# pandegroup/openmm

Measured on NVIDIA H100. Metric: ns/day, higher is better.
Workload: dtype f32

## Files before the change

### openmm_b200/csrc/engine.cu

```cuda
#include "engine.h"
#include "../../include/b200md.h"
#include <stdexcept>
#include <algorithm>
#include <cmath>
#include <cstring>
#include <cstdlib>
#include <map>
#include <set>
#include <dlfcn.h>
#include <thread>

static std::string g_create_error;

template <class T> struct DevBuf {
    T* p = nullptr; size_t n = 0; bool owned = true;
    void attach(void* ptr, size_t count) { free(); p = (T*) ptr; n = count; owned = false; }
    void alloc(size_t count) {
        if (!owned) { if (count > n) throw std::runtime_error("window buffer too small"); return; }
        free(); n = count; if (count) CUDA_CHECK(cudaMalloc(&p, count*sizeof(T)));
    }
    void upload(const std::vector<T>& v) { if (v.size() > n) alloc(v.size()); if (!v.empty()) CUDA_CHECK(cudaMemcpy(p, v.data(), v.size()*sizeof(T), cudaMemcpyHostToDevice)); }
    void zero() { if (n) CUDA_CHECK(cudaMemset(p, 0, n*sizeof(T))); }
    void free() { if (p && owned) cudaFree(p); p = nullptr; n = 0; owned = true; }
    ~DevBuf() { free(); }
// ... 19 lines not shown
        AllReduce = (decltype(AllReduce)) dlsym(lib, "ncclAllReduce");
        AllGather = (decltype(AllGather)) dlsym(lib, "ncclAllGather");
        CommDestroy = (decltype(CommDestroy)) dlsym(lib, "ncclCommDestroy");
        GetErrorString = (decltype(GetErrorString)) dlsym(lib, "ncclGetErrorString");
        if (!GetUniqueId || !CommInitRank || !AllReduce) { err = "libnccl lacks required symbols"; return false; }
        return true;
    }
};
static NcclApi g_nccl;
enum { NCCL_INT8 = 0, NCCL_INT64 = 4, NCCL_FLOAT32 = 7, NCCL_FLOAT64 = 8, NCCL_SUM = 0 };

struct b200md_ctx {
    int device = 0;
    int natoms = 0, npad = 0, nblocks = 0;
    bool finalized = false;
    std::string err;
    cudaStream_t stream = nullptr;
    cudaStream_t streamPme = nullptr;
    cudaStream_t streamBonded = nullptr;
    cudaEvent_t evFork = nullptr, evJoin = nullptr, evJoinBonded = nullptr;
    bool pmeOnly = false;
    bool listDirty = true;
    bool overlapPme = true;
    bool pmeBrick = true;
    int brickAtoms = 64, brickPoints = 8192;
    bool listBuilt = false;
    std::vector<double> mass, charge, sigma, epsilon;
    b200md_nonbonded_desc nbdesc{};
    bool haveNb = false;
    std::vector<int> excI, excJ; std::vector<double> excQQ, excSig, excEps;
    std::vector<int> bondI, bondJ; std::vector<double> bondR0, bondK;
    std::vector<int> angI, angJ, angK; std::vector<double> angT0, angKK;
    std::vector<int> torI, torJ, torK, torL, torN; std::vector<double> torPhase, torKK;
    std::vector<int> rbI, rbJ, rbK, rbL; std::vector<double> rbC;
    std::vector<int> cmapSize, cmapMap, cmapAtoms; std::vector<double> cmapCoeff;
    std::vector<unsigned char> bondGroup, angGroup, torGroup, rbGroup, cmapGroup;
    std::vector<int> conI, conJ; std::vector<double> conD;
    int cmFreq = 0;
    std::vector<int4> hUnitAtoms;
    double boxA[3] = {0, 0, 0}, boxB[3] = {0, 0, 0}, boxC[3] = {0, 0, 0};
    bool haveBox = false;
    bool haveOrigin = false;
    double padFrac = 0.10;
    DevBuf<float4> posq, velm, sposq[2], swrap[2], refPos, atomShift, blockCenter[2], blockHalf[2], superCenter[2], superHalf[2];
    DevBuf<float2> sigeps, ssigeps[2];
    DevBuf<double> chargeD; DevBuf<double2> sigepsD;
    DevBuf<long long> force;
    DevBuf<double> energy, cmScratch;
    DevBuf<int> molStart, molAtoms, cellOffset, sorig[2], sortedOf, cellRank, cellCount, cellFill, atomCell, tmpSorted, tileI[2], tileJ[2], tileMask[2], listCounters, counters, exclStart, exclList;
    DevBuf<unsigned int> maskPool[2];
    DevBuf<unsigned long long> stepCounter;
    DevBuf<unsigned int> blocksDone;
    bool stepStateValid = false;
    DevBuf<real> grid, eterm;
    DevBuf<long long> gridFixed;
    DevBuf<real2> cgrid;
    DevBuf<real2> tw[3];
    DevBuf<double> moduli[3];
    DevBuf<int2> bondAtoms, excAtoms; DevBuf<double2> bondParams, angleParams;
    DevBuf<int4> angleAtoms, torsionAtoms, unitAtoms; DevBuf<double4> torsionParams, excParams;
    DevBuf<int> unitType; DevBuf<float4> unitParams;
    DevBuf<unsigned char> bondGroupDev, angGroupDev, torGroupDev, rbGroupDev, cmapGroupDev;
    DevBuf<int4> rbAtoms, cmapAtomsDev; DevBuf<double> rbParams, cmapCoeffDev; DevBuf<int> cmapMapDev; DevBuf<int2> cmapMapsDev;
    std::vector<int> ccmaCons;
    DevBuf<int> ccCompCon, ccCompAtom, ccRowStart, ccCol, ccAtoms, ccAStart, ccACon;
    DevBuf<int2> ccConAtoms; DevBuf<float> ccDist, ccRedMass, ccVal, ccDelta1, ccDelta2;
    DevBuf<float4> ccRij, ccXold, ccXunc;
    int precision = B200MD_PRECISION_SINGLE;
    DevBuf<float4> posqCorr; DevBuf<double4> velmD, unitParamsD;
    DevBuf<double> ccDistD, ccRedMassD, ccDelta1D, ccDelta2D; DevBuf<double4> ccRijD, ccXoldD, ccXuncD, ccXposD;
    bool mixed() const { return precision == B200MD_PRECISION_MIXED; }
    CcmaDev ccma{};
    NbDev nb{};
    PmeDev pme{};
    BondedDev bd{};
    UnitDev units{};
    IntegDev integ{};
    bool haveIntegrator = false;
    double dt = 0, temperature = 0, friction = 0;
    double time = 0;
    int64_t stepCount = 0;
    double selfEnergy = 0, dispersionCoefficient = 0;
    int64_t forceEvals = 0, kernelLaunches = 0, graphInstantiations = 0;
    DevBuf<int> baroStart, baroAtoms;
    int baroNmol = 0;
    DevBuf<float4> savePosq, savePosqCorr; DevBuf<int> saveCellOffset; DevBuf<long long> saveForce;
    bool haveSaved = false;
    cudaGraphExec_t stepGraph = nullptr;
    cudaGraphExec_t multiGraph = nullptr;
    bool graphValid = false;
    bool multiValid = false;
    bool useGraph = true;
    int graphSteps = 8;
    int stepLaunches = 0;
    void* comm = nullptr;
    int rank = 0, world = 1;
    bool p2p = false;
    CommDev cd{};
    char* window = nullptr; size_t windowBytes = 0;
    void* peerMapped[B200MD_MAX_RANKS] = {nullptr};
    DevBuf<unsigned long long> commCounters;
    DevBuf<unsigned int> commDone;
    bool velStale = false;
    std::vector<float4> hbuf4, hcorr4;
    std::vector<int> hoffset;
    std::vector<long long> hforce;
};

#define API_BEGIN(ctx) if (!(ctx)) return -1; try { CUDA_CHECK(cudaSetDevice((ctx)->device));
#define API_END(ctx) } catch (std::exception& e) { (ctx)->err = e.what(); return -1; } return 0;

static void require(bool cond, const char* msg) { if (!cond) throw std::runtime_error(msg); }
static void check_flags(b200md_ctx* c);
static void sync_velocities(b200md_ctx* c);
static void sync_positions(b200md_ctx* c);

extern "C" const char* b200md_version(void) { return "b200md 0.2 (sm_90a)"; }
extern "C" const char* b200md_last_error(const b200md_ctx* ctx) { return ctx ? ctx->err.c_str() : g_create_error.c_str(); }

extern "C" int b200md_create(b200md_ctx** out, int device, int natoms) {
    try {
        require(out != nullptr && natoms > 0, "b200md_create: bad arguments");
        int count = 0;
        cudaError_t e = cudaGetDeviceCount(&count);
        if (e != cudaSuccess || count == 0)
            throw std::runtime_error(std::string("b200md_create: no CUDA device available (") + cudaGetErrorString(e) + "); this library has no CPU fallback");
        require(device >= 0 && device < count, "b200md_create: device index out of range");
        CUDA_CHECK(cudaSetDevice(device));
        b200md_ctx* c = new b200md_ctx();
        c->device = device;
        c->natoms = natoms;
        c->npad = ((natoms + 31)/32)*32;
        c->nblocks = c->npad/32;
        CUDA_CHECK(cudaStreamCreateWithFlags(&c->stream, cudaStreamNonBlocking));
        if (getenv("B200MD_NO_OVERLAP")) c->overlapPme = false;
        if (getenv("B200MD_PME_BRICK")) c->pmeBrick = atoi(getenv("B200MD_PME_BRICK")) != 0;
        if (getenv("B200MD_PME_BRICK_POINTS")) c->brickPoints = std::max(1, atoi(getenv("B200MD_PME_BRICK_POINTS")));
        int hi = 0;
        CUDA_CHECK(cudaDeviceGetStreamPriorityRange(nullptr, &hi));
        CUDA_CHECK(cudaStreamCreateWithPriority(&c->streamPme, cudaStreamNonBlocking, hi));
        CUDA_CHECK(cudaStreamCreateWithPriority(&c->streamBonded, cudaStreamNonBlocking, hi));
        CUDA_CHECK(cudaEventCreateWithFlags(&c->evFork, cudaEventDisableTiming));
        CUDA_CHECK(cudaEventCreateWithFlags(&c->evJoin, cudaEventDisableTiming));
        CUDA_CHECK(cudaEventCreateWithFlags(&c->evJoinBonded, cudaEventDisableTiming));
        c->mass.assign(natoms, 1.0);
        c->charge.assign(natoms, 0.0); c->sigma.assign(natoms, 1.0); c->epsilon.assign(natoms, 0.0);
        const char* pf = getenv("B200MD_PAD_FRACTION");
        if (pf) c->padFrac = atof(pf);
        const char* ug = getenv("B200MD_USE_GRAPH");
        if (ug) c->useGraph = atoi(ug) != 0;
        const char* gs = getenv("B200MD_GRAPH_STEPS");
        if (gs) c->graphSteps = std::max(1, atoi(gs));
        *out = c;
        return 0;
    } catch (std::exception& e) { g_create_error = e.what(); return -1; }
}

extern "C" void b200md_destroy(b200md_ctx* ctx) {
    if (!ctx) return;
    cudaSetDevice(ctx->device);
    cudaDeviceSynchronize();
    if (ctx->stepGraph) cudaGraphExecDestroy(ctx->stepGraph);
// ... 1201 lines not shown
        }
        else { CUDA_CHECK(cudaMemcpy(p, ctx->velm.p, sizeof(float4)*ctx->npad, cudaMemcpyDeviceToHost)); p += sizeof(float4)*ctx->npad; }
        CUDA_CHECK(cudaMemcpy(p, ctx->cellOffset.p, sizeof(int)*3*ctx->npad, cudaMemcpyDeviceToHost));
        return need;
    } catch (std::exception& e) { ctx->err = e.what(); return -1; }
}
extern "C" int b200md_checkpoint_load(b200md_ctx* ctx, const void* buf, int64_t size) {
    API_BEGIN(ctx)
    ctx->stepStateValid = false;
    require(ctx->finalized, "checkpoint_load before finalize");
    require(size >= (int64_t) sizeof(CkptHeader), "checkpoint blob too small");
    CkptHeader h; memcpy(&h, buf, sizeof(h));
    require(memcmp(h.magic, "B200MDCK", 8) == 0 && (h.version == 2 || h.version == 3) && h.natoms == ctx->natoms, "checkpoint blob does not match this context");
    require(h.version == ckpt_version(ctx), h.version == 3 ? "the checkpoint was written in mixed precision and this context is single precision"
                                                           : "the checkpoint was written in single precision and this context is mixed precision");
    require(size >= ckpt_bytes(ctx), "checkpoint blob too small");
    sync_positions(ctx);
    CUDA_CHECK(cudaStreamSynchronize(ctx->stream));
    ctx->time = h.time; ctx->stepCount = h.stepCount;
    for (int i = 0; i < 3; i++) { ctx->boxA[i] = h.box[i]; ctx->boxB[i] = h.box[3+i]; ctx->boxC[i] = h.box[6+i]; }
    const char* p = (const char*) buf + sizeof(h);
    CUDA_CHECK(cudaMemcpy(ctx->posq.p, p, sizeof(float4)*ctx->npad, cudaMemcpyHostToDevice)); p += sizeof(float4)*ctx->npad;
    if (ctx->mixed()) {
        CUDA_CHECK(cudaMemcpy(ctx->posqCorr.p, p, sizeof(float4)*ctx->npad, cudaMemcpyHostToDevice)); p += sizeof(float4)*ctx->npad;
        CUDA_CHECK(cudaMemcpy(ctx->velmD.p, p, sizeof(double4)*ctx->npad, cudaMemcpyHostToDevice)); p += sizeof(double4)*ctx->npad;
    }
    else { CUDA_CHECK(cudaMemcpy(ctx->velm.p, p, sizeof(float4)*ctx->npad, cudaMemcpyHostToDevice)); p += sizeof(float4)*ctx->npad; }
    CUDA_CHECK(cudaMemcpy(ctx->cellOffset.p, p, sizeof(int)*3*ctx->npad, cudaMemcpyHostToDevice));
    CUDA_CHECK(cudaMemcpy(ctx->stepCounter.p, &h.rngStep, sizeof(unsigned long long), cudaMemcpyHostToDevice));
    host_set_state(ctx); ctx->velStale = false;
    if (ctx->haveBox) apply_box(ctx);
    const int one = 1;
    CUDA_CHECK(cudaMemcpy(&ctx->counters.p[CT_REBUILD], &one, sizeof(int), cudaMemcpyHostToDevice)); ctx->listDirty = true;
    API_END(ctx)
}

static bool role_split(const b200md_ctx* c) { return c->world > 1 && c->comm && !c->p2p && c->nb.method == B200MD_NB_PME && c->haveNb; }
static NbDev role_nb(const b200md_ctx* c) {
    NbDev nb = c->nb;
    if (role_split(c)) {
        if (c->rank == c->world - 1) { nb.rank = 0; nb.world = 1; }
        else nb.world = c->world - 1;
    }
    return nb;
}

static PmeDev pme_for_launch(const b200md_ctx* c) {
    PmeDev p = c->pme;
    p.brickAtoms = (c->pmeBrick && c->world == 1 && !c->pmeOnly && c->listBuilt) ? c->brickAtoms : 0;
    p.brickPoints = c->brickPoints;
    return p;
}

static int enqueue_forces(b200md_ctx* c, int terms, bool energy, bool forcesAlreadyZero = false, bool inStep = false, unsigned int groupMask = 0xffffffffu) {
    int launches = 0;
    cudaStream_t s = c->stream;
    if (!forcesAlreadyZero) CUDA_CHECK(cudaMemsetAsync(c->force.p, 0, sizeof(long long)*3*c->npad, s));
    if (energy) CUDA_CHECK(cudaMemsetAsync(c->energy.p, 0, sizeof(double)*B200MD_NUM_ENERGY, s));
    bool direct = (terms & B200MD_TERM_NB_DIRECT) && c->haveNb;
    bool recip = (terms & B200MD_TERM_NB_RECIP) && c->haveNb && c->nb.method == B200MD_NB_PME;
    const bool split = role_split(c);
    const int pmeRank = c->world - 1;
    NbDev nbSave = c->nb;
    if (split) {
        if (c->rank == pmeRank) direct = false; else recip = false;
        c->nb = role_nb(c);
    }
    struct Restore { b200md_ctx* c; NbDev saved; ~Restore() { c->nb = saved; } } restore{c, nbSave};
    const bool p2p = c->p2p;
    const bool fork = direct && recip && c->overlapPme && !(c->world > 1 && c->comm && !p2p);
    cudaStream_t sp = fork ? c->streamPme : s;
    if (p2p && !direct) { launch_pos_wait(c->nb, c->cd, s); launches++; }
    const PmeDev pme = pme_for_launch(c);
    const bool forkAfterList = fork && direct && pme.brickAtoms > 0;
    auto launch_recip = [&]() {
        if (fork) {
            CUDA_CHECK(cudaEventRecord(c->evFork, s));
            CUDA_CHECK(cudaStreamWaitEvent(sp, c->evFork, 0));
        }
        if (recip) {
            launch_pme_spread(c->nb, pme, c->cd, sp); launches++;
            if (p2p) { launch_grid_push(c->pme, c->cd, sp); launches++; }
            else if (c->world > 1 && c->comm && !split) {
                int rc = g_nccl.AllReduce(c->gridFixed.p, c->gridFixed.p, (size_t) c->pme.nx*c->pme.ny*c->pme.nz, NCCL_INT64, NCCL_SUM, c->comm, sp);
                if (rc != 0) throw std::runtime_error("ncclAllReduce(grid) failed");
            }
            launch_pme_fft_conv(c->nb, c->pme, c->cd, energy && (split || p2p || c->rank == 0), fft_beside_tiles(c), sp); launches += pme_fft_launch_count(c->pme);
            launch_pme_gather(c->nb, pme, c->cd, sp); launches++;
        }
        if (fork) CUDA_CHECK(cudaEventRecord(c->evJoin, sp));
    };
    if (!forkAfterList) launch_recip();
    if (direct) {
        launch_check_displacement(c->nb, c->cd, s); launches++;
        launch_list_build(c->nb, s); launches += LIST_BUILD_LAUNCHES;
    }
    int bterms = terms & (B200MD_TERM_BONDS | B200MD_TERM_ANGLES | B200MD_TERM_TORSIONS | B200MD_TERM_RB_TORSIONS | B200MD_TERM_CMAP);
    if (c->haveNb) bterms |= terms & B200MD_TERM_NB_DIRECT;
    const int nbonded = c->bd.nbonds + c->bd.nangles + c->bd.ntorsions + c->bd.nrb + c->bd.ncmap + c->bd.nexc;
    const bool bonded = bterms && nbonded > 0 && !(split && c->rank == pmeRank);
    auto launch_bonded_terms = [&](cudaStream_t sb) { BondedDev bd = c->bd; bd.groupMask = groupMask; launch_bonded(c->nb, bd, bterms, energy, sb); launches++; };
    const bool forkBonded = forkAfterList && bonded;
    if (forkAfterList) launch_recip();
    if (forkBonded) {
        CUDA_CHECK(cudaStreamWaitEvent(c->streamBonded, c->evFork, 0));
        launch_bonded_terms(c->streamBonded);
        CUDA_CHECK(cudaEventRecord(c->evJoinBonded, c->streamBonded));
    }
    if (direct) { launch_pair(c->nb, energy, s); launches++; }
    if (bonded && !forkBonded) launch_bonded_terms(s);
    const bool pushEarly = p2p && fork;
    if (pushEarly) { launch_force_push(c->nb, c->cd, s); launches++; }
    if (fork) CUDA_CHECK(cudaStreamWaitEvent(s, c->evJoin, 0));
    if (forkBonded) CUDA_CHECK(cudaStreamWaitEvent(s, c->evJoinBonded, 0));
    if (p2p) {
        if (!pushEarly) { launch_force_push(c->nb, c->cd, s); launches++; }
        if (!inStep) { launch_force_total(c->nb, c->cd, s); launches += 2; }
    }
    if (c->world > 1 && c->comm) {
        int rc = 0;
        if (!p2p) rc = g_nccl.AllReduce(c->force.p, c->force.p, (size_t) 3*c->npad, NCCL_INT64, NCCL_SUM, c->comm, s);
        if (rc != 0) throw std::runtime_error("ncclAllReduce(force) failed");
        if (energy) {
            rc = g_nccl.AllReduce(c->energy.p, c->energy.p, B200MD_NUM_ENERGY, NCCL_FLOAT64, NCCL_SUM, c->comm, s);
            if (rc != 0) throw std::runtime_error("ncclAllReduce(energy) failed");
        }
    }
    CUDA_CHECK(cudaGetLastError());
    return launches;
}

static void check_flags(b200md_ctx* c) {
    if (!c->finalized) return;
    int h[8];
    CUDA_CHECK(cudaMemcpyAsync(h, c->counters.p, sizeof(int)*8, cudaMemcpyDeviceToHost, c->stream));
    CUDA_CHECK(cudaStreamSynchronize(c->stream));
    if (h[CT_OVERFLOW] == 2) throw std::runtime_error("B200 platform: neighbour-list construction timed out at a grid barrier (k_list_prep)");
    if (h[CT_OVERFLOW] == 3) throw std::runtime_error("B200 platform: multi-GPU exchange timed out waiting for a peer rank (every rank must issue the same sequence of calls)");
    if (h[CT_OVERFLOW]) throw std::runtime_error("B200 platform: neighbour-list tile capacity exceeded (" + std::to_string(c->nb.maxTiles) + " tiles) during the preceding steps; the trajectory since the last state read is invalid");
}

static bool role_split(const b200md_ctx* c);
static NbDev role_nb(const b200md_ctx* c);
static void invalidate_graph(b200md_ctx* c);

static void prepare_list(b200md_ctx* c) {
    if (!c->listDirty || !c->haveNb) { c->listDirty = false; return; }
// ... 31 lines not shown

extern "C" int b200md_compute(b200md_ctx* ctx, int terms, int want_forces, double* energy) {
    return b200md_compute_groups(ctx, terms, 0xffffffffu, want_forces, energy);
}

extern "C" int b200md_compute_groups(b200md_ctx* ctx, int terms, unsigned int bonded_group_mask, int want_forces, double* energy) {
    API_BEGIN(ctx)
    ctx->stepStateValid = false;
    (void) want_forces;
    require(ctx->finalized, "compute before finalize");
    const bool wantE = energy != nullptr;
    prepare_list(ctx);
    ctx->kernelLaunches += enqueue_forces(ctx, terms, wantE, false, false, bonded_group_mask);
    ctx->forceEvals++;
    if (wantE) {
        double h[B200MD_NUM_ENERGY];
        CUDA_CHECK(cudaMemcpyAsync(h, ctx->energy.p, sizeof(h), cudaMemcpyDeviceToHost, ctx->stream));
        check_flags(ctx);
        double e = 0;
        if (terms & B200MD_TERM_BONDS) e += h[EN_BOND];
        if (terms & B200MD_TERM_ANGLES) e += h[EN_ANGLE];
        if (terms & B200MD_TERM_TORSIONS) e += h[EN_TORSION];
        if (terms & B200MD_TERM_RB_TORSIONS) e += h[EN_RBTORSION];
        if (terms & B200MD_TERM_CMAP) e += h[EN_CMAP];
        if (ctx->haveNb) {
            if (terms & B200MD_TERM_NB_DIRECT) {
                e += h[EN_NB] + h[EN_EXC];
                const int m = ctx->nb.method;
                if (m == B200MD_NB_CUTOFF_PERIODIC || m == B200MD_NB_PME)
                    e += ctx->dispersionCoefficient/ctx->nb.box.volume;
            }
            if ((terms & B200MD_TERM_NB_RECIP) && ctx->nb.method == B200MD_NB_PME) e += h[EN_RECIP] + ctx->selfEnergy;
        }
        *energy = e;
    }
    API_END(ctx)
}

extern "C" int b200md_set_integrator(b200md_ctx* ctx, int kind, double dt, double temperature, double friction, int seed, double tol) {
    API_BEGIN(ctx)
    require(kind >= 0 && kind <= 2, "unknown integrator kind");
    IntegDev& in = ctx->integ;
    in.kind = kind; in.dt = (float) dt; in.tol = (float) tol; in.seed = (unsigned int) seed;
    const double kT = B200MD_BOLTZ*temperature;
    in.kT = (float) kT;
    const double vscale = std::exp(-dt*friction);
    in.vscale = (float) vscale;
    in.fscale = (float) (friction == 0 ? dt : (1-vscale)/friction);
    in.noisescale = (float) (kind == B200MD_INT_LANGEVIN_MIDDLE ? std::sqrt(1-vscale*vscale) : std::sqrt(kT*(1-vscale*vscale)));
    in.dtD = dt; in.tolD = tol; in.kTD = kT; in.vscaleD = vscale;
    in.fscaleD = friction == 0 ? dt : (1-vscale)/friction;
    in.noisescaleD = kind == B200MD_INT_LANGEVIN_MIDDLE ? std::sqrt(1-vscale*vscale) : std::sqrt(kT*(1-vscale*vscale));
    in.stepCounter = ctx->stepCounter.p;
    in.fused = 0; in.cmEveryStep = 0; in.cmScratch = ctx->cmScratch.p; in.blocksDone = ctx->blocksDone.p;
    ctx->dt = dt; ctx->temperature = temperature; ctx->friction = friction;
    ctx->haveIntegrator = true;
    invalidate_graph(ctx);
    API_END(ctx)
}

static int enqueue_step(b200md_ctx* c) {
    int launches = enqueue_forces(c, B200MD_TERM_ALL, false, true, true);
    IntegDev in = c->integ;
    in.fused = 1;
    in.cmEveryStep = (c->cmFreq == 1) ? 1 : 0;
    in.cmScratch = c->cmScratch.p;
    in.blocksDone = c->blocksDone.p;
    if (c->ccma.ncomp > 0) { launch_ccma_step(c->nb, c->ccma, in, c->stream); launches += 1; }
    launch_integrate(c->nb, c->units, in, c->cd, c->stream); launches += 1;
    return launches;
}

extern "C" int b200md_integrate_only(b200md_ctx* ctx) {
    API_BEGIN(ctx)
    ctx->stepStateValid = false;
    require(ctx->finalized && ctx->haveIntegrator, "integrate before finalize / set_integrator");
    if (ctx->ccma.ncomp > 0) launch_ccma_step(ctx->nb, ctx->ccma, ctx->integ, ctx->stream);
    launch_integrate(ctx->nb, ctx->units, ctx->integ, ctx->cd, ctx->stream);
    ctx->kernelLaunches += 2;
    ctx->velStale = ctx->p2p;
    ctx->time += ctx->dt; ctx->stepCount++;
    CUDA_CHECK(cudaGetLastError());
    API_END(ctx)
}

static void capture_steps(b200md_ctx* c, int nsteps, cudaGraphExec_t* exec, int* launches) {
    cudaGraph_t g;
    CUDA_CHECK(cudaStreamBeginCapture(c->stream, cudaStreamCaptureModeThreadLocal));
    int l = 0;
    try { for (int k = 0; k < nsteps; k++) l += enqueue_step(c); } catch (...) { cudaStreamEndCapture(c->stream, &g); throw; }
    CUDA_CHECK(cudaStreamEndCapture(c->stream, &g));
    *launches = l;
    if (*exec) {
        cudaGraphExecUpdateResultInfo info;
        if (cudaGraphExecUpdate(*exec, g, &info) == cudaSuccess) { cudaGraphDestroy(g); return; }
        (void) cudaGetLastError();
    }
    if (*exec) { cudaGraphExecDestroy(*exec); *exec = nullptr; }
    const cudaError_t e = cudaGraphInstantiate(exec, g, c->world == 1 ? cudaGraphInstantiateFlagUseNodePriority : 0);
    cudaGraphDestroy(g);
    CUDA_CHECK(e);
    c->graphInstantiations++;
}

extern "C" int b200md_step(b200md_ctx* ctx, int nsteps) {
    API_BEGIN(ctx)
    require(ctx->finalized && ctx->haveIntegrator, "step before finalize / set_integrator");
    b200md_ctx* c = ctx;
    int remaining = nsteps;
    prepare_list(c);
    if (!c->stepStateValid) {
        CUDA_CHECK(cudaMemsetAsync(c->force.p, 0, sizeof(long long)*3*c->npad, c->stream));
        if (c->cmFreq == 1) {
            IntegDev in = c->integ;
            in.cmScratch = c->cmScratch.p;
            sync_velocities(c);
            launch_cm_prime(c->nb, in, c->cd, c->stream);
        }
        c->stepStateValid = true;
    }
    while (remaining > 0) {
        if (c->cmFreq > 1 && c->stepCount % c->cmFreq == 0) { sync_velocities(c); launch_remove_cm(c->nb, c->cmScratch.p, c->stream); c->kernelLaunches += 2; }
        int done = 1;
        if (c->useGraph) {
            int untilCm = (c->cmFreq > 1) ? (int) (c->cmFreq - c->stepCount % c->cmFreq) : remaining;
            if (c->graphSteps > 1 && remaining >= c->graphSteps && untilCm >= c->graphSteps) {
                if (!c->multiValid) { int l; capture_steps(c, c->graphSteps, &c->multiGraph, &l); c->stepLaunches = l/c->graphSteps; c->multiValid = true; }
                CUDA_CHECK(cudaGraphLaunch(c->multiGraph, c->stream));
                done = c->graphSteps;
            }
            else {
                if (!c->graphValid) { capture_steps(c, 1, &c->stepGraph, &c->stepLaunches); c->graphValid = true; }
                CUDA_CHECK(cudaGraphLaunch(c->stepGraph, c->stream));
            }
            c->kernelLaunches += (int64_t) c->stepLaunches*done;
        }
        else
            c->kernelLaunches += enqueue_step(c);
        c->velStale = c->p2p;
        c->forceEvals += done;
        c->stepCount += done;
        c->time += c->dt*done;
        remaining -= done;
    }
    CUDA_CHECK(cudaGetLastError());
    API_END(ctx)
}

extern "C" int b200md_kinetic_energy(b200md_ctx* ctx, double* ke) {
    API_BEGIN(ctx)
    require(ctx->finalized, "kinetic_energy before finalize");
    const bool shifted = ctx->haveIntegrator && ctx->integ.kind != B200MD_INT_LANGEVIN_MIDDLE;
    const double shift = !shifted ? 0.0 : ctx->mixed() ? 0.5*ctx->integ.dtD : (double) (0.5f*ctx->integ.dt);
    sync_positions(ctx); sync_velocities(ctx);
    CUDA_CHECK(cudaMemsetAsync(ctx->energy.p + EN_KE, 0, sizeof(double), ctx->stream));
    launch_kinetic_energy(ctx->nb, ctx->units, ctx->integ, shift, ctx->stream);
    launch_ccma_kinetic(ctx->nb, ctx->ccma, shift, 1e-4f, ctx->stream);
    ctx->kernelLaunches++;
    CUDA_CHECK(cudaMemcpyAsync(ke, ctx->energy.p + EN_KE, sizeof(double), cudaMemcpyDeviceToHost, ctx->stream));
    check_flags(ctx);
    API_END(ctx)
}
extern "C" int b200md_apply_constraints(b200md_ctx* ctx, double tol) {
    API_BEGIN(ctx)
    sync_positions(ctx);
    launch_constrain_positions(ctx->nb, ctx->units, tol, ctx->stream);
    launch_ccma_apply(ctx->nb, ctx->ccma, false, tol, ctx->stream);
    ctx->kernelLaunches++;
    CUDA_CHECK(cudaStreamSynchronize(ctx->stream));
    API_END(ctx)
}
extern "C" int b200md_apply_velocity_constraints(b200md_ctx* ctx, double tol) {
    API_BEGIN(ctx)
    ctx->stepStateValid = false;
    sync_positions(ctx); sync_velocities(ctx);
    launch_constrain_velocities(ctx->nb, ctx->units, tol, ctx->stream);
    launch_ccma_apply(ctx->nb, ctx->ccma, true, tol, ctx->stream);
    ctx->kernelLaunches++;
    CUDA_CHECK(cudaStreamSynchronize(ctx->stream));
    API_END(ctx)
}

extern "C" int b200md_comm_unique_id(void* id128) {
    std::string err;
    if (!g_nccl.load(err)) { g_create_error = err; return -1; }
    return g_nccl.GetUniqueId(id128) == 0 ? 0 : -1;
}
extern "C" int b200md_comm_init(b200md_ctx* ctx, int rank, int world, const void* id128) {
    API_BEGIN(ctx)
    require(!ctx->finalized, "comm_init must precede finalize");
    require(!ctx->mixed() || world <= 1, "comm_init: mixed precision is not supported in multi-GPU runs (use Precision=single)");
    std::string err;
    if (!g_nccl.load(err)) throw std::runtime_error(err);
    NcclApi::Uid uid; memcpy(uid.b, id128, 128);
    int rc = g_nccl.CommInitRank(&ctx->comm, world, uid, rank);
    if (rc != 0) throw std::runtime_error(std::string("ncclCommInitRank failed: ") + (g_nccl.GetErrorString ? g_nccl.GetErrorString(rc) : "?"));
    ctx->rank = rank; ctx->world = world;
    DevBuf<long long> warm; warm.alloc(64); warm.zero();
// ... 170 lines not shown
```

### openmm_b200/csrc/engine.h

```cpp
#pragma once
#include <cuda_runtime.h>
#include <stdint.h>
#include <stdexcept>
#include <string>
#include <vector>

#define B200MD_TILE 32
#define B200MD_PME_ORDER 5
#define B200MD_FORCE_SCALE 4294967296.0
#define B200MD_ONE_4PI_EPS0 138.93545764438198
#define B200MD_BOLTZ 0.00831446261815324
#define B200MD_MAX_RADIX 16
#define B200MD_MAX_FFT_STAGES 8

#define CUDA_CHECK(x) do { cudaError_t e_ = (x); if (e_ != cudaSuccess) throw std::runtime_error(std::string(#x) + ": " + cudaGetErrorString(e_)); } while (0)

template <typename... P, typename... A>
inline void launch_high(void (*kernel)(P...), dim3 grid, dim3 block, size_t smem, cudaStream_t s, A... args) {
    static const int hi = [] { int lo = 0, h = 0; cudaDeviceGetStreamPriorityRange(&lo, &h); return h; }();
    cudaLaunchAttribute at[1];
    at[0].id = cudaLaunchAttributePriority;
    at[0].val.priority = hi;
    cudaLaunchConfig_t cfg = {};
    cfg.gridDim = grid; cfg.blockDim = block; cfg.dynamicSmemBytes = smem; cfg.stream = s;
// ... 92 lines not shown
    bool smPartition;
    float closeCut2;
};

enum { EN_NB = 0, EN_RECIP = 1, EN_BOND = 2, EN_ANGLE = 3, EN_TORSION = 4, EN_EXC = 5, EN_KE = 6, EN_RBTORSION = 7, EN_CMAP = 8,
       B200MD_NUM_ENERGY = 9 };

struct PmeDev {
    int nx, ny, nz, nzc;
    real* grid;
    long long* gridFixed;
    real2* cgrid;
    real* eterm;
    const double* moduli[3];
    FftPlanDev plan[3];
    double alpha;
    int brickAtoms;
    int brickPoints;
};

struct BondedDev {
    int nbonds, nangles, ntorsions, nrb, ncmap, nexc;
    const int2* bondAtoms; const double2* bondParams;
    const int4* angleAtoms; const double2* angleParams;
    const int4* torsionAtoms; const double4* torsionParams;
    const int4* rbAtoms; const double* rbParams;
    const int4* cmapAtoms; const int* cmapMap; const int2* cmapMaps; const double* cmapCoeff;
    const int2* excAtoms; const double4* excParams;
    int excPeriodic;
    const unsigned char* bondGroup; const unsigned char* angleGroup; const unsigned char* torsionGroup;
    const unsigned char* rbGroup; const unsigned char* cmapGroup;
    unsigned int groupMask;
};

struct UnitDev {
    int nunits;
    const int4* unitAtoms;
    const int* unitType;
    const float4* unitParams;
    const double4* unitParamsD;
};

struct IntegDev {
    int kind;
    float dt, vscale, fscale, noisescale;
    float kT;
    float tol;
    double dtD, vscaleD, fscaleD, noisescaleD, kTD, tolD;
    unsigned int seed;
    unsigned long long stepIndex;
    unsigned long long* stepCounter;
    int fused;
    int cmEveryStep;
    double* cmScratch;
    unsigned int* blocksDone;
};

#define B200MD_MAX_RANKS 8
enum { CH_POS = 0,
       CH_FORCE = 1,
       CH_FINAL = 2,
       CH_GRID = 3,
       CH_FWD = 4,
       CH_INV = 5,
       CH_POT = 6,
       CH_VEL = 7,
       CH_COUNT = 8 };
struct CommDev {
    int rank, world;
    int atomLo[B200MD_MAX_RANKS + 1];
    int unitLo[B200MD_MAX_RANKS + 1];
    int xLo[B200MD_MAX_RANKS + 1];
    int lineChunk;
    int maxPlanes;
    char* peer[B200MD_MAX_RANKS];
    size_t offFlags, offPosq, offVelm, offForce, offFinbox, offCm, offGridInbox, offLineBuf, offPlaneBuf, offGrid;
    unsigned long long* epoch;
    unsigned long long* posNeed;
    unsigned int* done;
    int* errFlag;
    int posByPush;
};

#ifdef __CUDACC__
__device__ __forceinline__ unsigned long long ld_acquire_sys(const unsigned long long* p) {
    unsigned long long v;
    asm volatile("ld.acquire.sys.global.u64 %0, [%1];" : "=l"(v) : "l"(p) : "memory");
    return v;
}
__device__ __forceinline__ void st_release_sys(unsigned long long* p, unsigned long long v) {
    asm volatile("st.release.sys.global.u64 [%0], %1;" :: "l"(p), "l"(v) : "memory");
}
__device__ __forceinline__ unsigned long long* comm_flag(const CommDev& cd, int onRank, int ch, int src) {
    return (unsigned long long*) (cd.peer[onRank] + cd.offFlags) + ch*B200MD_MAX_RANKS + src;
}
__device__ __forceinline__ void comm_wait(const CommDev& cd, int ch, unsigned long long need) {
    if (cd.world > 1 && need != 0ull) {
        if (threadIdx.x < cd.world && (int) threadIdx.x != cd.rank && threadIdx.y == 0 && threadIdx.z == 0) {
            const unsigned long long* f = comm_flag(cd, cd.rank, ch, threadIdx.x);
            long spins = 0;
            while (ld_acquire_sys(f) < need) {
                if (*((volatile int*) cd.errFlag) == 3) break;
                __nanosleep(64);
                if (++spins > (1L << 22)) { *cd.errFlag = 3; break; }
            }
        }
// ... 191 lines not shown
```

### openmm_b200/csrc/integrate.cu

```cuda
#include "engine.h"
#include <algorithm>
#include "../../include/b200md.h"

template <class R> struct V3 { R x, y, z; };
template <class R> __device__ __forceinline__ V3<R> operator+(V3<R> a, V3<R> b) { return {a.x+b.x, a.y+b.y, a.z+b.z}; }
template <class R> __device__ __forceinline__ V3<R> operator-(V3<R> a, V3<R> b) { return {a.x-b.x, a.y-b.y, a.z-b.z}; }
template <class R> __device__ __forceinline__ V3<R> operator*(V3<R> a, R s) { return {a.x*s, a.y*s, a.z*s}; }
template <class R> __device__ __forceinline__ R dot(V3<R> a, V3<R> b) { return a.x*b.x + a.y*b.y + a.z*b.z; }

template <class R>
__device__ void settle_positions(const V3<R>* x, V3<R>* d, const R* m, R dist1, R dist2) {
    const V3<R> xp0 = d[0], xp1 = d[1], xp2 = d[2];
    const R xb0 = x[1].x-x[0].x, yb0 = x[1].y-x[0].y, zb0 = x[1].z-x[0].z;
    const R xc0 = x[2].x-x[0].x, yc0 = x[2].y-x[0].y, zc0 = x[2].z-x[0].z;
    const R invTotalMass = R(1)/(m[0]+m[1]+m[2]);
    const R xcom = (xp0.x*m[0] + (xb0+xp1.x)*m[1] + (xc0+xp2.x)*m[2])*invTotalMass;
    const R ycom = (xp0.y*m[0] + (yb0+xp1.y)*m[1] + (yc0+xp2.y)*m[2])*invTotalMass;
    const R zcom = (xp0.z*m[0] + (zb0+xp1.z)*m[1] + (zc0+xp2.z)*m[2])*invTotalMass;
    const R xa1 = xp0.x - xcom, ya1 = xp0.y - ycom, za1 = xp0.z - zcom;
    const R xb1 = xb0 + xp1.x - xcom, yb1 = yb0 + xp1.y - ycom, zb1 = zb0 + xp1.z - zcom;
    const R xc1 = xc0 + xp2.x - xcom, yc1 = yc0 + xp2.y - ycom, zc1 = zc0 + xp2.z - zcom;
    const R xaksZd = yb0*zc0 - zb0*yc0, yaksZd = zb0*xc0 - xb0*zc0, zaksZd = xb0*yc0 - yb0*xc0;
    const R xaksXd = ya1*zaksZd - za1*yaksZd, yaksXd = za1*xaksZd - xa1*zaksZd, zaksXd = xa1*yaksZd - ya1*xaksZd;
    const R xaksYd = yaksZd*zaksXd - zaksZd*yaksXd, yaksYd = zaksZd*xaksXd - xaksZd*zaksXd, zaksYd = xaksZd*yaksXd - yaksZd*xaksXd;
// ... 111 lines not shown
    V3<R> x[4], v[4], f[4];
    R invM[4], m[4];
    R4<R> prm;
};

template <class R> __device__ R4<R> unit_params(const UnitDev& un, int u);
template <> __device__ __forceinline__ float4 unit_params<float>(const UnitDev& un, int u) { return un.unitParams[u]; }
template <> __device__ __forceinline__ double4 unit_params<double>(const UnitDev& un, int u) { return un.unitParamsD[u]; }

template <class R>
__device__ __forceinline__ bool load_unit(const NbDev& nb, const UnitDev& un, int u, Unit<R>& U, bool wantForce, const CommDev* cd = nullptr) {
    const int4 at = un.unitAtoms[u];
    U.atom[0] = at.x; U.atom[1] = at.y; U.atom[2] = at.z; U.atom[3] = at.w;
    U.type = un.unitType[u];
    U.prm = unit_params<R>(un, u);
    U.n = 0;
#pragma unroll
    for (int k = 0; k < 4; k++) {
        const int a = U.atom[k];
        if (a < 0) continue;
        U.n = k+1;
        const R4<R> p = load_pos<R>(nb, a);
        const R4<R> v = vel_array<R>(nb)[a];
        U.x[k] = {p.x, p.y, p.z};
        U.v[k] = {v.x, v.y, v.z};
        U.invM[k] = v.w;
        U.m[k] = (v.w > R(0)) ? R(1)/v.w : R(0);
        if (wantForce) {
            long long fx = nb.force[a], fy = nb.force[a + nb.npad], fz = nb.force[a + 2*nb.npad];
            if (cd != nullptr && cd->world > 1) {
                const long long* in = (const long long*) (cd->peer[cd->rank] + cd->offFinbox);
                for (int q = 0; q < cd->world; q++) if (q != cd->rank) {
                    const long long* iq = in + (size_t) q*3*nb.npad;
                    fx += iq[a]; fy += iq[a + nb.npad]; fz += iq[a + 2*nb.npad];
                }
            }
            U.f[k] = {fixed_to_real<R>(fx), fixed_to_real<R>(fy), fixed_to_real<R>(fz)};
        }
    }
    return true;
}

template <class R>
__device__ __forceinline__ void constrain_pos(const Unit<R>& U, V3<R>* d, R tol) {
    if (U.type == 1) settle_positions(U.x, d, U.m, U.prm.x, U.prm.y);
    else if (U.type == 2) { const R dist[3] = {U.prm.x, U.prm.y, U.prm.z}; shake_positions(U.x, d, U.invM, dist, U.n-1, tol); }
}
template <class R>
__device__ __forceinline__ void constrain_vel(const Unit<R>& U, V3<R>* v, R tol) {
    if (U.type == 1) settle_velocities(U.x, v, U.m);
    else if (U.type == 2) shake_velocities(U.x, v, U.invM, U.n-1, tol);
}

template <int KIND, class R>
__global__ void __launch_bounds__(128, sizeof(R) == 8 ? 1 : 0) k_integrate(NbDev nb, UnitDev un, IntegDev in, CommDev cd) {
    const bool multi = cd.world > 1;
    const bool useInbox = multi && in.fused;
    const unsigned long long E = multi ? *cd.epoch + 1ull : 0ull;
    if (useInbox) comm_wait(cd, CH_FORCE, E);
    const int u = (multi ? cd.unitLo[cd.rank] : 0) + blockIdx.x*blockDim.x + threadIdx.x;
    const bool active = u < (multi ? cd.unitLo[cd.rank + 1] : un.nunits);
    const unsigned long long step = *in.stepCounter;
    const IntegR<R> ic = integ_r<R>(in);
    Unit<R> U;
    U.n = 0;
    V3<R> d[4];
    const R invDt = R(1)/ic.dt;
    const bool cmFused = in.fused && in.cmEveryStep;
    V3<R> vcm = {R(0), R(0), R(0)};
    if (cmFused) {
        double c[4];
        if (multi) {
            const double* t = (const double*) (cd.peer[cd.rank] + cd.offCm) + 4*(step % 3ull);
            c[0] = c[1] = c[2] = c[3] = 0.0;
            for (int q = 0; q < cd.world; q++) for (int k = 0; k < 4; k++) c[k] += t[q*12 + k];
        }
        else { const double* t = in.cmScratch + 4*(step % 3ull); c[0] = t[0]; c[1] = t[1]; c[2] = t[2]; c[3] = t[3]; }
        const double im = (c[3] > 0.0) ? 1.0/c[3] : 0.0;
        vcm = {(R) (c[0]*im), (R) (c[1]*im), (R) (c[2]*im)};
    }
    if (active) {
    load_unit(nb, un, u, U, true, useInbox ? &cd : nullptr);
    if (in.fused) {
        _Pragma("unroll") for (int k = 0; k < 4; k++) if (k < U.n) {
            const int a = U.atom[k];
            nb.force[a] = 0; nb.force[a + nb.npad] = 0; nb.force[a + 2*nb.npad] = 0;
            if (U.invM[k] > R(0)) U.v[k] = U.v[k] - vcm;
        }
    }
    if (KIND == B200MD_INT_LANGEVIN_MIDDLE) {
        _Pragma("unroll") for (int k = 0; k < 4; k++) if (k < U.n) U.v[k] = U.v[k] + U.f[k]*(ic.dt*U.invM[k]);
        constrain_vel(U, U.v, ic.tol);
        V3<R> du[4];
        _Pragma("unroll") for (int k = 0; k < 4; k++) if (k < U.n) {
            d[k] = U.v[k]*(R(0.5)*ic.dt);
            if (U.invM[k] > R(0)) {
                const float3 g = gauss3(in.seed, U.atom[k], step);
                const R ns = ic.noisescale*sqrt_r(ic.kT*U.invM[k]);
                U.v[k] = U.v[k]*ic.vscale + V3<R>{g.x, g.y, g.z}*ns;
            }
            d[k] = d[k] + U.v[k]*(R(0.5)*ic.dt);
            if (U.invM[k] == R(0)) d[k] = {R(0), R(0), R(0)};
            du[k] = d[k];
        }
        constrain_pos(U, d, ic.tol);
        _Pragma("unroll") for (int k = 0; k < 4; k++) if (k < U.n) U.v[k] = U.v[k] + (d[k] - du[k])*invDt;
    }
    else {
        _Pragma("unroll") for (int k = 0; k < 4; k++) if (k < U.n) {
            V3<R> vn;
            if (KIND == B200MD_INT_LANGEVIN) {
                vn = U.v[k]*ic.vscale + U.f[k]*(ic.fscale*U.invM[k]);
                if (U.invM[k] > R(0) && ic.noisescale > R(0)) {
                    const float3 g = gauss3(in.seed, U.atom[k], step);
                    vn = vn + V3<R>{g.x, g.y, g.z}*(ic.noisescale*sqrt_r(U.invM[k]));
                }
            }
            else
                vn = U.v[k] + U.f[k]*(ic.dt*U.invM[k]);
            if (U.invM[k] == R(0)) vn = U.v[k];
            d[k] = (U.invM[k] == R(0)) ? V3<R>{R(0), R(0), R(0)} : vn*ic.dt;
        }
        constrain_pos(U, d, ic.tol);
        _Pragma("unroll") for (int k = 0; k < 4; k++) if (k < U.n) if (U.invM[k] > R(0)) U.v[k] = d[k]*invDt;
    }
    _Pragma("unroll") for (int k = 0; k < 4; k++) if (k < U.n) {
        const int a = U.atom[k];
        store_pos<R>(nb, a, U.x[k].x + d[k].x, U.x[k].y + d[k].y, U.x[k].z + d[k].z);
        vel_array<R>(nb)[a] = make_r4(U.v[k].x, U.v[k].y, U.v[k].z, U.invM[k]);
        if (multi && !cd.posByPush) {
            const float4 pn = nb.posq[a];
            for (int k = 1; k < cd.world; k++) {
                const int q = (cd.rank + k) % cd.world;
                ((float4*) (cd.peer[q] + cd.offPosq))[a] = pn;
            }
        }
    }
    }
    if (!in.fused && !(multi && !cd.posByPush)) return;
    if (cmFused) {
        double px = 0, py = 0, pz = 0, m = 0;
        _Pragma("unroll") for (int k = 0; k < 4; k++) if (k < U.n && U.invM[k] > R(0)) {
            const double mk = U.m[k];
            px += mk*U.v[k].x; py += mk*U.v[k].y; pz += mk*U.v[k].z; m += mk;
        }
        for (int off = 16; off > 0; off >>= 1) {
            px += __shfl_xor_sync(0xffffffffu, px, off); py += __shfl_xor_sync(0xffffffffu, py, off);
            pz += __shfl_xor_sync(0xffffffffu, pz, off); m += __shfl_xor_sync(0xffffffffu, m, off);
        }
        __shared__ double red[4][4];
        if ((threadIdx.x & 31) == 0) { red[threadIdx.x >> 5][0] = px; red[threadIdx.x >> 5][1] = py; red[threadIdx.x >> 5][2] = pz; red[threadIdx.x >> 5][3] = m; }
        __syncthreads();
        if (threadIdx.x < 4) {
            double t = 0;
            for (int w = 0; w < (int) (blockDim.x >> 5); w++) t += red[w][threadIdx.x];
            atomicAdd(&in.cmScratch[4*((step + 1ull) % 3ull) + threadIdx.x], t);
            if (blockIdx.x == 0) in.cmScratch[4*((step + 2ull) % 3ull) + threadIdx.x] = 0.0;
        }
    }
    if (multi && !cd.posByPush) {
        const bool lastBlock = comm_arrive(cd, CH_POS, gridDim.x);
        if (lastBlock && threadIdx.x == 0) {
            if (cmFused) {
                const double* mine = in.cmScratch + 4*((step + 1ull) % 3ull);
                for (int q = 0; q < cd.world; q++) {
                    double* t = (double*) (cd.peer[q] + cd.offCm) + cd.rank*12 + 4*((step + 1ull) % 3ull);
                    for (int k = 0; k < 4; k++) t[k] = ((volatile const double*) mine)[k];
                }
            }
            comm_publish(cd, CH_POS, E);
            *cd.posNeed = E;
            *cd.epoch = E;
            *in.stepCounter = step + 1ull;
        }
        return;
    }
    __shared__ int last;
    __syncthreads();
    if (threadIdx.x == 0) {
        __threadfence();
        last = (atomicAdd(in.blocksDone, 1u) == gridDim.x - 1);
    }
    __syncthreads();
    if (last && threadIdx.x == 0) {
        *in.blocksDone = 0u;
        *in.stepCounter = step + 1ull;
    }
}

__global__ void k_step_advance(IntegDev in) { *in.stepCounter += 1ull; }

template <class R>
__global__ void __launch_bounds__(256) k_cm_prime(NbDev nb, IntegDev in, double* table) {
    const unsigned long long step = *in.stepCounter;
    double* c = table + 4*(step % 3ull);
    const int a = blockIdx.x*blockDim.x + threadIdx.x;
    double px = 0, py = 0, pz = 0, m = 0;
    if (a < nb.natoms) {
        const R4<R> v = vel_array<R>(nb)[a];
        if (v.w > R(0)) { m = 1.0/v.w; px = m*v.x; py = m*v.y; pz = m*v.z; }
    }
    for (int off = 16; off > 0; off >>= 1) {
        px += __shfl_xor_sync(0xffffffffu, px, off); py += __shfl_xor_sync(0xffffffffu, py, off);
        pz += __shfl_xor_sync(0xffffffffu, pz, off); m += __shfl_xor_sync(0xffffffffu, m, off);
    }
    __shared__ double red[8][4];
    if ((threadIdx.x & 31) == 0) { red[threadIdx.x >> 5][0] = px; red[threadIdx.x >> 5][1] = py; red[threadIdx.x >> 5][2] = pz; red[threadIdx.x >> 5][3] = m; }
    __syncthreads();
    if (threadIdx.x < 4) {
        double t = 0;
        for (int w = 0; w < 8; w++) t += red[w][threadIdx.x];
        atomicAdd(&c[threadIdx.x], t);
    }
}

void launch_cm_prime(const NbDev& nb, const IntegDev& integ, const CommDev& cd, cudaStream_t s) {
    cudaMemsetAsync(integ.cmScratch, 0, 12*sizeof(double), s);
    double* table = integ.cmScratch;
    if (cd.world > 1) {
        table = (double*) (cd.peer[cd.rank] + cd.offCm);
        cudaMemsetAsync(table, 0, (size_t) B200MD_MAX_RANKS*12*sizeof(double), s);
    }
    if (nb.velmD) k_cm_prime<double><<<(nb.natoms + 255)/256, 256, 0, s>>>(nb, integ, table);
    else k_cm_prime<float><<<(nb.natoms + 255)/256, 256, 0, s>>>(nb, integ, table);
}

template <int KIND>
static void launch_integrate_kind(int grid, const NbDev& nb, const UnitDev& units, const IntegDev& integ, const CommDev& cd, cudaStream_t s) {
    if (nb.velmD) k_integrate<KIND, double><<<grid, 64, 0, s>>>(nb, units, integ, cd);
    else k_integrate<KIND, float><<<grid, 64, 0, s>>>(nb, units, integ, cd);
}

void launch_integrate(const NbDev& nb, const UnitDev& units, const IntegDev& integ, const CommDev& cd, cudaStream_t s) {
    const int n = cd.world > 1 ? cd.unitLo[cd.rank + 1] - cd.unitLo[cd.rank] : units.nunits;
    const int grid = std::max(1, (n + 63)/64);
    if (integ.kind == B200MD_INT_VERLET) launch_integrate_kind<B200MD_INT_VERLET>(grid, nb, units, integ, cd, s);
    else if (integ.kind == B200MD_INT_LANGEVIN) launch_integrate_kind<B200MD_INT_LANGEVIN>(grid, nb, units, integ, cd, s);
    else launch_integrate_kind<B200MD_INT_LANGEVIN_MIDDLE>(grid, nb, units, integ, cd, s);
    if (!integ.fused && (cd.world <= 1 || cd.posByPush)) k_step_advance<<<1, 1, 0, s>>>(integ);
// ... 155 lines not shown
```

Baseline: 1341.

## Fold neighbor-list displacement check into the integrate kernel

Moves the per-step displacement check and sorted-position refresh into the integration kernel, which runs per constraint unit, whenever there is a single rank, a nonbonded force and no CCMA. In-step force evaluation then skips its separate check-displacement launch. One standalone check still runs at the start of each step call, and the last block resets the list counters. This removes a kernel launch and a pass over positions each step, at the cost of extra work in the integrator and a more fragile coupling of list state to it.

```diff
diff --git a/openmm_b200/csrc/engine.cu b/openmm_b200/csrc/engine.cu
--- a/openmm_b200/csrc/engine.cu
+++ b/openmm_b200/csrc/engine.cu
@@ -95,6 +95,7 @@
     DevBuf<unsigned long long> stepCounter;
     DevBuf<unsigned int> blocksDone;
     bool stepStateValid = false;
+    bool listChecked = false;
     DevBuf<real> grid, eterm;
     DevBuf<long long> gridFixed;
     DevBuf<real2> cgrid;
@@ -150,7 +151,7 @@
     std::vector<long long> hforce;
 };
 
-#define API_BEGIN(ctx) if (!(ctx)) return -1; try { CUDA_CHECK(cudaSetDevice((ctx)->device));
+#define API_BEGIN(ctx) if (!(ctx)) return -1; (ctx)->listChecked = false; try { CUDA_CHECK(cudaSetDevice((ctx)->device));
 #define API_END(ctx) } catch (std::exception& e) { (ctx)->err = e.what(); return -1; } return 0;
 
 static void require(bool cond, const char* msg) { if (!cond) throw std::runtime_error(msg); }
@@ -1458,6 +1459,10 @@
     return p;
 }
 
+static bool fold_check(const b200md_ctx* c) {
+    return c->world == 1 && c->haveNb && c->ccma.ncomp == 0;
+}
+
 static int enqueue_forces(b200md_ctx* c, int terms, bool energy, bool forcesAlreadyZero = false, bool inStep = false, unsigned int groupMask = 0xffffffffu) {
     int launches = 0;
     cudaStream_t s = c->stream;
@@ -1498,7 +1503,7 @@
     };
     if (!forkAfterList) launch_recip();
     if (direct) {
-        launch_check_displacement(c->nb, c->cd, s); launches++;
+        if (!(inStep && fold_check(c))) { launch_check_displacement(c->nb, c->cd, s); launches++; }
         launch_list_build(c->nb, s); launches += LIST_BUILD_LAUNCHES;
     }
     int bterms = terms & (B200MD_TERM_BONDS | B200MD_TERM_ANGLES | B200MD_TERM_TORSIONS | B200MD_TERM_RB_TORSIONS | B200MD_TERM_CMAP);
@@ -1636,7 +1641,7 @@
     in.fscaleD = friction == 0 ? dt : (1-vscale)/friction;
     in.noisescaleD = kind == B200MD_INT_LANGEVIN_MIDDLE ? std::sqrt(1-vscale*vscale) : std::sqrt(kT*(1-vscale*vscale));
     in.stepCounter = ctx->stepCounter.p;
-    in.fused = 0; in.cmEveryStep = 0; in.cmScratch = ctx->cmScratch.p; in.blocksDone = ctx->blocksDone.p;
+    in.fused = 0; in.cmEveryStep = 0; in.checkList = 0; in.cmScratch = ctx->cmScratch.p; in.blocksDone = ctx->blocksDone.p;
     ctx->dt = dt; ctx->temperature = temperature; ctx->friction = friction;
     ctx->haveIntegrator = true;
     invalidate_graph(ctx);
@@ -1650,6 +1655,7 @@
     in.cmEveryStep = (c->cmFreq == 1) ? 1 : 0;
     in.cmScratch = c->cmScratch.p;
     in.blocksDone = c->blocksDone.p;
+    in.checkList = fold_check(c) ? 1 : 0;
     if (c->ccma.ncomp > 0) { launch_ccma_step(c->nb, c->ccma, in, c->stream); launches += 1; }
     launch_integrate(c->nb, c->units, in, c->cd, c->stream); launches += 1;
     return launches;
@@ -1688,6 +1694,7 @@
 }
 
 extern "C" int b200md_step(b200md_ctx* ctx, int nsteps) {
+    const bool checked = ctx && ctx->listChecked;
     API_BEGIN(ctx)
     require(ctx->finalized && ctx->haveIntegrator, "step before finalize / set_integrator");
     b200md_ctx* c = ctx;
@@ -1703,6 +1710,8 @@
         }
         c->stepStateValid = true;
     }
+    const bool fold = fold_check(c);
+    if (fold && !checked) { launch_check_displacement(c->nb, c->cd, c->stream); c->kernelLaunches++; }
     while (remaining > 0) {
         if (c->cmFreq > 1 && c->stepCount % c->cmFreq == 0) { sync_velocities(c); launch_remove_cm(c->nb, c->cmScratch.p, c->stream); c->kernelLaunches += 2; }
         int done = 1;
@@ -1728,6 +1737,7 @@
         remaining -= done;
     }
     CUDA_CHECK(cudaGetLastError());
+    c->listChecked = fold;
     API_END(ctx)
 }
 
diff --git a/openmm_b200/csrc/engine.h b/openmm_b200/csrc/engine.h
--- a/openmm_b200/csrc/engine.h
+++ b/openmm_b200/csrc/engine.h
@@ -168,6 +168,7 @@
     unsigned long long* stepCounter;
     int fused;
     int cmEveryStep;
+    int checkList;
     double* cmScratch;
     unsigned int* blocksDone;
 };
diff --git a/openmm_b200/csrc/integrate.cu b/openmm_b200/csrc/integrate.cu
--- a/openmm_b200/csrc/integrate.cu
+++ b/openmm_b200/csrc/integrate.cu
@@ -187,6 +187,27 @@
     else if (U.type == 2) shake_velocities(U.x, v, U.invM, U.n-1, tol);
 }
 
+template <class R>
+__device__ __forceinline__ void check_moved_unit(const NbDev& nb, const Unit<R>& U) {
+    float4 p[4], r[4];
+    int s[4];
+    _Pragma("unroll") for (int k = 0; k < 4; k++) if (k < U.n) {
+        const int a = U.atom[k];
+        p[k] = nb.posq[a]; r[k] = nb.refPos[a]; s[k] = nb.sortedOf[a];
+    }
+    const ListDev& L = nb.list[nb.counters[CT_CUR] & 1];
+    bool moved = false;
+    _Pragma("unroll") for (int k = 0; k < 4; k++) if (k < U.n) {
+        const float dx = p[k].x-r[k].x, dy = p[k].y-r[k].y, dz = p[k].z-r[k].z;
+        const float d2 = dx*dx + dy*dy + dz*dz;
+        moved |= !(d2 <= nb.halfPad2);
+        L.sposq[s[k]] = p[k];
+        if (s[k] == nb.natoms - 1)
+            for (int t = nb.natoms; t < nb.npad; t++) L.sposq[t] = make_float4(p[k].x, p[k].y, p[k].z, 0.f);
+    }
+    if (moved) nb.counters[CT_REBUILD] = 1;
+}
+
 template <int KIND, class R>
 __global__ void __launch_bounds__(128, sizeof(R) == 8 ? 1 : 0) k_integrate(NbDev nb, UnitDev un, IntegDev in, CommDev cd) {
     const bool multi = cd.world > 1;
@@ -271,6 +292,7 @@
             }
         }
     }
+    if (in.checkList) check_moved_unit<R>(nb, U);
     }
     if (!in.fused && !(multi && !cd.posByPush)) return;
     if (cmFused) {
@@ -320,6 +342,7 @@
     if (last && threadIdx.x == 0) {
         *in.blocksDone = 0u;
         *in.stepCounter = step + 1ull;
+        if (in.checkList) { nb.counters[CT_CURSOR] = 0; nb.counters[CT_PAIRSTART] = 0; }
     }
 }
 
```

Result: faster. 1356, median of 6 (+1.1%).
